# Tycro-Games/Raytracer-VoxPopuli

Measured on AMD Instinct MI355X. Metric: Mray/s (primary+shadow) at 1920×1080, 1024³ world; 1/2/4/8-GPU, higher is better.
Workload: dtype f32

## Files before the change

include/vpx.h:

```cpp
#ifndef VPX_H_
#define VPX_H_

#include <stddef.h>
#include <stdint.h>

#ifdef __cplusplus
extern "C" {
#endif

#define VPX_ABI_VERSION 2

#define VPX_OK 0
#define VPX_E_INVALID (-1)
#define VPX_E_DEVICE (-2)
#define VPX_E_NOMEM (-3)
#define VPX_E_STATE (-4)

#define VPX_MAT_NON_METAL_WHITE 0
#define VPX_MAT_NON_METAL_PINK 4
#define VPX_MAT_METAL_HIGH 5
#define VPX_MAT_METAL_LOW 7
#define VPX_MAT_GLASS 8
#define VPX_MAT_SMOKE_LOW_DENSITY 9
#define VPX_MAT_SMOKE_PLAYER 14
// ... 118 lines not shown
const char* vpx_last_error(const vpx_ctx* ctx);
int vpx_abi_version(void);
int vpx_set_stream(vpx_ctx* ctx, void* hip_stream);
int vpx_synchronize(vpx_ctx* ctx);
int vpx_set_pipeline(vpx_ctx* ctx, uint32_t depth);

int vpx_upload_grid(vpx_ctx* ctx, uint32_t grid_id, const uint8_t* cells, uint32_t n);
int vpx_generate_tiled_grid(vpx_ctx* ctx, uint32_t grid_id, uint32_t n, const uint8_t* model,
                            uint32_t mx, uint32_t my, uint32_t mz,
                            uint32_t px, uint32_t py, uint32_t pz, uint32_t ground);
int vpx_grid_fill(vpx_ctx* ctx, uint32_t grid_id, uint8_t value);
int vpx_grid_write_box(vpx_ctx* ctx, uint32_t grid_id, const uint8_t* src, uint32_t x0, uint32_t y0,
                       uint32_t z0, uint32_t dx, uint32_t dy, uint32_t dz);
int vpx_grid_emissive_sphere(vpx_ctx* ctx, uint32_t grid_id, uint8_t mat, float radius);
int vpx_grid_checksum(vpx_ctx* ctx, uint32_t grid_id, uint64_t* out);
int vpx_grid_axis_planes(vpx_ctx* ctx, uint32_t grid_id, uint16_t* out, uint64_t count);
int vpx_set_volumes(vpx_ctx* ctx, const vpx_volume* volumes, uint32_t count);
int vpx_set_materials(vpx_ctx* ctx, const vpx_material* materials, uint32_t count);
int vpx_set_lights(vpx_ctx* ctx,
                   const vpx_point_light* points, uint32_t n_points,
                   const vpx_spot_light* spots, uint32_t n_spots,
                   const vpx_area_light* areas, uint32_t n_areas,
                   const vpx_dir_light* dir);
int vpx_set_shapes(vpx_ctx* ctx, const vpx_sphere* spheres, uint32_t n_spheres,
                   const vpx_triangle* triangles, uint32_t n_triangles);
int vpx_set_camera(vpx_ctx* ctx, const vpx_camera* camera);
int vpx_set_sky(vpx_ctx* ctx, const float* rgb, uint32_t width, uint32_t height,
                float hdr_contribution);

#define VPX_ARITH_EXACT 0u
// ... 104 lines not shown
```

raytracer-voxpopuli_amd/abi.py:

```python
import ctypes as C
import os

import numpy as np

HERE = os.path.dirname(os.path.abspath(__file__))
LIB_PATH = os.path.join(HERE, "libvpx_hip.so")
ABI_VERSION = 2

VPX_OK = 0
VPX_E_INVALID, VPX_E_DEVICE, VPX_E_NOMEM, VPX_E_STATE = -1, -2, -3, -4
VPX_FLAG_AA = 0x1
VPX_FLAG_DOF = 0x2
VPX_FLAG_NO_TONEMAP = 0x4
VPX_ARITH_EXACT, VPX_ARITH_X86_HOST = 0, 1
VPX_FLAG_SKY = 0x8
MAT_NONE = 255
SKY_DEFAULT = (0.392, 0.584, 0.829)

f3 = C.c_float * 3


class Volume(C.Structure):
    _fields_ = [("grid_id", C.c_uint32), ("reserved", C.c_uint32), ("matrix", C.c_float * 16),
                ("inv_matrix", C.c_float * 16), ("b0", f3), ("b1", f3)]
# ... 102 lines not shown
    "vpx_create": (C.c_int, [C.c_int, C.POINTER(C.c_void_p)]),
    "vpx_create_multi": (C.c_int, [C.POINTER(C.c_int), C.c_int, C.POINTER(C.c_void_p)]),
    "vpx_destroy": (C.c_int, [C.c_void_p]),
    "vpx_last_error": (C.c_char_p, [C.c_void_p]),
    "vpx_abi_version": (C.c_int, []),
    "vpx_set_stream": (C.c_int, [C.c_void_p, C.c_void_p]),
    "vpx_synchronize": (C.c_int, [C.c_void_p]),
    "vpx_set_pipeline": (C.c_int, [C.c_void_p, C.c_uint32]),
    "vpx_gl_register_buffer": (C.c_int, [C.c_void_p, C.c_uint]),
    "vpx_gl_map": (C.c_int, [C.c_void_p, C.POINTER(C.c_void_p), C.POINTER(C.c_size_t)]),
    "vpx_gl_unmap": (C.c_int, [C.c_void_p]),
    "vpx_upload_grid": (C.c_int, [C.c_void_p, C.c_uint32, C.c_void_p, C.c_uint32]),
    "vpx_generate_tiled_grid": (C.c_int, [C.c_void_p, C.c_uint32, C.c_uint32, C.c_void_p] + [C.c_uint32] * 7),
    "vpx_grid_checksum": (C.c_int, [C.c_void_p, C.c_uint32, C.POINTER(C.c_uint64)]),
    "vpx_grid_axis_planes": (C.c_int, [C.c_void_p, C.c_uint32, C.c_void_p, C.c_uint64]),
    "vpx_set_volumes": (C.c_int, [C.c_void_p, C.POINTER(Volume), C.c_uint32]),
    "vpx_set_materials": (C.c_int, [C.c_void_p, C.POINTER(Material), C.c_uint32]),
    "vpx_set_lights": (C.c_int, [C.c_void_p, C.POINTER(PointLight), C.c_uint32, C.POINTER(SpotLight), C.c_uint32,
                                 C.POINTER(AreaLight), C.c_uint32, C.POINTER(DirLight)]),
    "vpx_set_shapes": (C.c_int, [C.c_void_p, C.POINTER(Sphere), C.c_uint32, C.POINTER(Triangle), C.c_uint32]),
    "vpx_set_camera": (C.c_int, [C.c_void_p, C.POINTER(Camera)]),
    "vpx_set_sky": (C.c_int, [C.c_void_p, C.c_void_p, C.c_uint32, C.c_uint32, C.c_float]),
    "vpx_render": (C.c_int, [C.c_void_p, C.POINTER(FrameParams), C.c_void_p, C.c_void_p, C.POINTER(Stats)]),
    "vpx_render_tiles": (C.c_int, [C.c_void_p, C.POINTER(FrameParams), C.c_uint32, C.c_uint32, C.c_uint32,
                                   C.c_uint32, C.c_void_p, C.POINTER(Stats)]),
    "vpx_render_tiles_accum": (C.c_int, [C.c_void_p, C.POINTER(FrameParams), C.c_uint32, C.c_uint32, C.c_uint32,
                                         C.c_uint32, C.c_void_p, C.c_void_p, C.POINTER(Stats)]),
    "vpx_composite_rgb8": (C.c_int, [C.c_void_p, C.POINTER(FrameParams), C.c_uint32, C.c_uint32, C.c_uint32,
                                     C.c_void_p, C.c_void_p]),
    "vpx_render_window": (C.c_int, [C.c_void_p, C.POINTER(FrameParams), C.c_uint32, C.c_void_p, C.c_void_p]),
# ... 87 lines not shown
```

raytracer-voxpopuli_amd/context.py:

```python
import ctypes as C

import numpy as np

from . import abi


class Context:
    def __init__(self, device=0, devices=None):
        self.lib = abi.load_library()
        h = C.c_void_p()
        if devices is not None:
            arr = (C.c_int * len(devices))(*[int(d) for d in devices])
            rc = self.lib.vpx_create_multi(arr, len(devices), C.byref(h))
            if rc != abi.VPX_OK:
                raise abi.VpxError(f"vpx_create_multi(devices={list(devices)}) failed ({rc})")
            device = int(devices[0])
        else:
            rc = self.lib.vpx_create(int(device), C.byref(h))
            if rc != abi.VPX_OK:
                raise abi.VpxError(f"vpx_create(device={device}) failed ({rc}): no usable HIP device")
        self.h = h
        self.device = device
        self.devices = list(devices) if devices is not None else [device]
        self.scene = None
# ... 78 lines not shown
        self._chk(self.lib.vpx_grid_emissive_sphere(self.h, grid_id, int(mat), float(radius)),
                  "vpx_grid_emissive_sphere")

    def grid_checksum(self, grid_id=0):
        out = C.c_uint64()
        self._chk(self.lib.vpx_grid_checksum(self.h, grid_id, C.byref(out)), "vpx_grid_checksum")
        return out.value

    def grid_axis_planes(self, grid_id, n):
        nb2 = ((n + 3) // 4 + 3) // 4
        out = np.zeros((24, 64 * nb2 ** 3), np.uint16)
        self._chk(self.lib.vpx_grid_axis_planes(self.h, grid_id, out.ctypes.data_as(C.c_void_p), out.size),
                  "vpx_grid_axis_planes")
        return out

    def render(self, params, accum_ptr, rgb_ptr=None, stats=False):
        st = abi.Stats() if stats else None
        self._chk(self.lib.vpx_render(self.h, C.byref(params), C.c_void_p(accum_ptr), C.c_void_p(rgb_ptr or 0),
                                      C.byref(st) if st is not None else None), "vpx_render")
        return st

    def render_reproject(self, params, prev, history_ptr, rgb_ptr=None, stats=False):
        st = abi.Stats() if stats else None
        self._chk(self.lib.vpx_render_reproject(self.h, C.byref(params), C.byref(prev), C.c_void_p(history_ptr),
                                                C.c_void_p(rgb_ptr or 0), C.byref(st) if st is not None else None),
                  "vpx_render_reproject")
        return st

    def render_tiles(self, params, rank, n_ranks, packed_ptr, stats=False, tile=16):
        st = abi.Stats() if stats else None
# ... 104 lines not shown
```

raytracer-voxpopuli_amd/csrc/vpx_kernels.hip:

```cpp
#include <hip/hip_runtime.h>
#include <hip/hip_gl_interop.h>
#include <rccl/rccl.h>

#include <algorithm>
#include <cmath>
#include <cstdio>
#include <cstdlib>
#include <cstring>
#include <string>
#include <array>
#include <atomic>
#include <vector>

#include "vpx_wavefront.hpp"

using namespace vpx;

namespace {

constexpr int kTile = 16;
#ifndef VPX_SPLIT_PRIMARY
#define VPX_SPLIT_PRIMARY 1
#endif
#ifndef VPX_DEFER_INSTANCES
// ... 332 lines not shown
                               uint32_t nb3, uint8_t* __restrict__ dfp) {
    const uint64_t plane = (uint64_t)nb2 * nb2 * nb2 * 64;
    for (uint64_t s = (uint64_t)blockIdx.x * blockDim.x + threadIdx.x; s < plane; s += (uint64_t)gridDim.x * blockDim.x) {
        const uint64_t parent = s >> 6;
        const uint32_t j = (uint32_t)(s & 63u);
        const uint32_t bx = (uint32_t)(parent % nb2) * 4 + (j & 3u);
        const uint32_t by = (uint32_t)((parent / nb2) % nb2) * 4 + ((j >> 2) & 3u);
        const uint32_t bz = (uint32_t)(parent / ((uint64_t)nb2 * nb2)) * 4 + (j >> 4);
        const bool occ = (l2[skip::blk_index(bx >> 2, by >> 2, bz >> 2, nb3)] >> ((bx & 3u) | ((by & 3u) << 2) | ((bz & 3u) << 4))) & 1ull;
        const uint64_t m = occ ? 0ull : l1[s];
#pragma unroll
        for (uint32_t o = 0; o < 8; ++o) dfp[o * plane + s] = (uint8_t)(m >> (8 * o));
    }
}

__global__ void build_axis_k(const uint8_t* __restrict__ dfp, uint32_t nb1, uint32_t nb2, uint16_t* __restrict__ dfa) {
    const uint64_t plane = (uint64_t)nb2 * nb2 * nb2 * 64;
    const uint64_t total = plane * 24;
    for (uint64_t t = (uint64_t)blockIdx.x * blockDim.x + threadIdx.x; t < total; t += (uint64_t)gridDim.x * blockDim.x) {
        const uint32_t oa = (uint32_t)(t / plane);
        const uint64_t s = t - (uint64_t)oa * plane;
        const uint32_t o = oa / 3u, a = oa - o * 3u;
        const uint64_t parent = s >> 6;
        const uint32_t j = (uint32_t)(s & 63u);
        const uint32_t bx = (uint32_t)(parent % nb2) * 4 + (j & 3u);
        const uint32_t by = (uint32_t)((parent / nb2) % nb2) * 4 + ((j >> 2) & 3u);
        const uint32_t bz = (uint32_t)(parent / ((uint64_t)nb2 * nb2)) * 4 + (j >> 4);
        const uint8_t* pl = dfp + (uint64_t)o * plane;
        const uint32_t k = pl[s];
        auto cube = [&](uint32_t x, uint32_t y, uint32_t z) -> uint32_t { return pl[skip::blk_index(x, y, z, nb2)]; };
        dfa[t] = k ? (uint16_t)(k | skip::axis_len(bx, by, bz, o, a, k, nb1, cube) << 8) : (uint16_t)0;
    }
}

__global__ void write_box_k(uint8_t* __restrict__ grid, uint32_t n, const uint8_t* __restrict__ src, uint32_t x0,
                            uint32_t y0, uint32_t z0, uint32_t dx, uint32_t dy, uint32_t dz) {
    const uint64_t total = (uint64_t)dx * dy * dz;
    const uint64_t n64 = n;
    for (uint64_t i = (uint64_t)blockIdx.x * blockDim.x + threadIdx.x; i < total; i += (uint64_t)gridDim.x * blockDim.x) {
        const uint64_t x = i % dx, y = (i / dx) % dy, z = i / ((uint64_t)dx * dy);
        grid[(x0 + x) + (y0 + y) * n64 + (z0 + z) * n64 * n64] = src[i];
    }
}

__global__ void emissive_sphere_k(uint8_t* __restrict__ grid, uint32_t n, uint8_t mat, float radius, uint32_t x0,
                                  uint32_t cnt) {
// ... 854 lines not shown
        VPX_HIP(c, sync_all(c));
        (void)hipFree(g.ptr);
        (void)hipFree(g.l1);
        (void)hipFree(g.l2);
        (void)hipFree(g.dfp);
        g.ptr = nullptr, g.l1 = nullptr, g.l2 = nullptr, g.dfp = nullptr;
    }
    g.n = n;
    g.nb1 = (n + 3) / 4;
    g.nb2 = (g.nb1 + 3) / 4;
    g.nb3 = (g.nb2 + 3) / 4;
    if (!g.ptr) {
        VPX_HIP(c, hipMalloc(&g.ptr, bytes));
        VPX_HIP(c, hipMalloc(&g.l1, sizeof(uint64_t) * (size_t)g.nb2 * g.nb2 * g.nb2 * 64));
        VPX_HIP(c, hipMalloc(&g.l2, sizeof(uint64_t) * (size_t)g.nb3 * g.nb3 * g.nb3 * 64));
        VPX_HIP(c, hipMalloc(&g.dfp, (8 + 2 * 24) * g.plane()));
    }
    return sync_grids(c);
}

static int build_df(vpx_ctx* c, const vpx_ctx::GridBuf& g) {
    const uint64_t threads = (uint64_t)g.nb1 * g.nb1 * 8;
    const unsigned blocks = (unsigned)((threads + 255) / 256);
    for (uint32_t s = 3 * (g.nb1 - 1) + 1; s-- > 0;) {
        hipLaunchKernelGGL(df_plane_k, dim3(blocks), dim3(256), 0, c->stream, (uint8_t*)g.l1, g.l2, g.nb1, g.nb2, g.nb3, s);
        VPX_HIP(c, hipGetLastError());
    }
    hipLaunchKernelGGL(build_planes_k, dim3(2048), dim3(256), 0, c->stream, g.l1, g.l2, g.nb2, g.nb3, g.dfp);
    VPX_HIP(c, hipGetLastError());
    hipLaunchKernelGGL(build_axis_k, dim3(8192), dim3(256), 0, c->stream, g.dfp, g.nb1, g.nb2, (uint16_t*)(g.dfp + 8 * g.plane()));
    VPX_HIP(c, hipGetLastError());
    return VPX_OK;
}

static int build_masks(vpx_ctx* c, uint32_t id) {
    auto& g = c->grids[id];
    hipLaunchKernelGGL(build_l1_k, dim3(2048), dim3(256), 0, c->stream, g.ptr, g.n, g.nb1, g.nb2, g.l1);
    VPX_HIP(c, hipGetLastError());
    hipLaunchKernelGGL(build_up_k, dim3(512), dim3(256), 0, c->stream, g.l1, g.nb2, g.nb3, g.l2);
    VPX_HIP(c, hipGetLastError());
    if (int r = build_df(c, g)) return r;
    VPX_HIP(c, sync_all(c));
    return VPX_OK;
}

// ... 105 lines not shown
int vpx_grid_checksum(vpx_ctx* c, uint32_t id, uint64_t* out) {
    VPX_GROUP_FIRST(c, vpx_grid_checksum(m_, id, out));
    if (!c || !out) return fail(c, VPX_E_INVALID, "null argument");
    if (id >= c->grids.size() || !c->grids[id].ptr) return fail(c, VPX_E_INVALID, "unknown grid");
    const uint64_t count = (uint64_t)c->grids[id].n * c->grids[id].n * c->grids[id].n;
    VPX_HIP(c, hipMemsetAsync(c->d_sum, 0, sizeof(unsigned long long), c->stream));
    hipLaunchKernelGGL(checksum_k, dim3(2048), dim3(256), 0, c->stream, c->grids[id].ptr, count, c->d_sum);
    VPX_HIP(c, hipGetLastError());
    unsigned long long h = 0;
    VPX_HIP(c, hipMemcpyAsync(&h, c->d_sum, sizeof(h), hipMemcpyDeviceToHost, c->stream));
    VPX_HIP(c, sync_all(c));
    *out = (uint64_t)h;
    return VPX_OK;
}

int vpx_grid_axis_planes(vpx_ctx* c, uint32_t id, uint16_t* out, uint64_t count) {
    VPX_GROUP_FIRST(c, vpx_grid_axis_planes(m_, id, out, count));
    if (!c || !out) return fail(c, VPX_E_INVALID, "null argument");
    if (id >= c->grids.size() || !c->grids[id].ptr) return fail(c, VPX_E_INVALID, "unknown grid");
    const auto& g = c->grids[id];
    if (count > 24 * g.plane()) return fail(c, VPX_E_INVALID, "more words than the axis planes hold");
    VPX_HIP(c, hipMemcpyAsync(out, g.dfp + 8 * g.plane(), count * sizeof(uint16_t), hipMemcpyDeviceToHost, c->stream));
    VPX_HIP(c, sync_all(c));
    return VPX_OK;
}

struct VolBox {
    float4 lo, hi;
};
static VolBox volume_bounds(const vpx_volume& v) {
    const float* m = v.inv_matrix;
    const double a[3][3] = {{m[0], m[1], m[2]}, {m[4], m[5], m[6]}, {m[8], m[9], m[10]}};
    const double det = a[0][0] * (a[1][1] * a[2][2] - a[1][2] * a[2][1]) -
                       a[0][1] * (a[1][0] * a[2][2] - a[1][2] * a[2][0]) +
                       a[0][2] * (a[1][0] * a[2][1] - a[1][1] * a[2][0]);
    const VolBox none{make_float4(-INFINITY, -INFINITY, -INFINITY, 0.f), make_float4(INFINITY, INFINITY, INFINITY, 0.f)};
    if (!(std::fabs(det) > 1e-30)) return none;
    double r[3][3];
// ... 940 lines not shown
```

raytracer-voxpopuli_amd/csrc/vpx_skip.hpp:

```cpp
#pragma once

#include <stdint.h>

#ifndef __HIP_DEVICE_COMPILE__
#include <cstring>
#endif

#if defined(__HIPCC__)
#define VPX_HD __host__ __device__ __forceinline__
#else
#define VPX_HD inline
#endif

namespace vpx {
namespace skip {

VPX_HD uint32_t fbits(float f) {
#if defined(__HIP_DEVICE_COMPILE__)
    return __float_as_uint(f);
#else
    uint32_t u;
    std::memcpy(&u, &f, 4);
    return u;
#endif
// ... 167 lines not shown

}
}

namespace vpx {
namespace skip {

struct GridView {
    const uint8_t* cells;
    const uint64_t* l1;
    const uint64_t* l2;
    uint32_t n, nb1, nb2, nb3;
    const uint8_t* dfp;
    uint64_t plane;
    const uint16_t* dfa;
};

struct Walk {
    uint32_t X, Y, Z;
    float t, tx, ty, tz;
    float dx, dy, dz;
    int32_t sx, sy, sz;
    uint32_t osh;
    uint64_t m1, m2;
};

VPX_HD void walk_begin(Walk& w) {
    w.m1 = w.m2 = 0ull;
    w.osh = ((w.sx < 0 ? 1u : 0u) | (w.sy < 0 ? 2u : 0u) | (w.sz < 0 ? 4u : 0u)) * 8u;
}
// ... 65 lines not shown
    const uint32_t bx = w.X >> 2, by = w.Y >> 2, bz = w.Z >> 2, np = g.nb2;
#if defined(__HIP_DEVICE_COMPILE__)
    const uint32_t parent = opar + __umul24(bz >> 2, __umul24(np, np)) + __umul24(by >> 2, np) + (bx >> 2);
#else
    const uint32_t parent = opar + (bz >> 2) * np * np + (by >> 2) * np + (bx >> 2);
#endif
    const uint64_t i = (uint64_t)parent << 6 | ((bx & 3u) | ((by & 3u) << 2) | ((bz & 3u) << 4));
#if defined(__HIP_DEVICE_COMPILE__)
    const uint32_t k = ((const __attribute__((address_space(1))) uint8_t*)g.dfp)[i];
#else
    const uint32_t k = g.dfp[i];
#endif
    return classify_dfp_byte<MINC>(w, g, k);
}
VPX_HD uint32_t plane_parent(const GridView& g, uint32_t o) { return o * (g.nb2 * g.nb2 * g.nb2); }
VPX_HD uint32_t dom_axis(const Walk& w) {
    return w.dx <= w.dy ? (w.dx <= w.dz ? 0u : 2u) : (w.dy <= w.dz ? 1u : 2u);
}
template <uint32_t MINC = kMinCube, uint32_t MINL = 2>
VPX_HD int classify_axis_o(Walk& w, const GridView& g, uint32_t apar) {
    const uint32_t bx = w.X >> 2, by = w.Y >> 2, bz = w.Z >> 2, np = g.nb2;
#if defined(__HIP_DEVICE_COMPILE__)
    const uint32_t parent = apar + __umul24(bz >> 2, __umul24(np, np)) + __umul24(by >> 2, np) + (bx >> 2);
#else
    const uint32_t parent = apar + (bz >> 2) * np * np + (by >> 2) * np + (bx >> 2);
#endif
    const uint64_t i = (uint64_t)parent << 6 | ((bx & 3u) | ((by & 3u) << 2) | ((bz & 3u) << 4));
#if defined(__HIP_DEVICE_COMPILE__)
    const uint32_t kl = ((const __attribute__((address_space(1))) uint16_t*)g.dfa)[i];
#else
    const uint32_t kl = g.dfa[i];
#endif
    if (kl == 0u) {
        w.m1 = load_mask(g.l1, blk_index(bx, by, bz, np));
        const uint32_t cb = (w.X & 3u) | ((w.Y & 3u) << 2) | ((w.Z & 3u) << 4);
        return ((w.m1 >> cb) & 1ull) ? 0 : 1;
    }
    w.m1 = kl;
    return (((kl & 255u) >= MINC) | ((kl >> 8) >= MINL)) ? 2 : 3;
}
VPX_HD uint32_t len_dfa(const Walk& w) { return ((uint32_t)w.m1 >> 8) & 255u; }
VPX_HD uint32_t cube_l1(const Walk& w) { return (uint32_t)(w.m1 >> w.osh) & 255u; }
VPX_HD uint32_t cube_dfp(const Walk& w) { return (uint32_t)w.m1 & 255u; }
VPX_HD void df_box(const Walk& w, uint32_t n, uint32_t k, uint32_t lo[3], uint32_t hi[3]) {
    const uint32_t k4 = k * 4u;
    const uint32_t c[3] = {w.X, w.Y, w.Z};
    const int32_t sg[3] = {w.sx, w.sy, w.sz};
    for (int k = 0; k < 3; ++k) {
        const uint32_t b = c[k] & ~3u;
        const uint32_t up = b + k4 - 1u, dn = b + 4u > k4 ? b + 4u - k4 : 0u;
        lo[k] = sg[k] > 0 ? c[k] : dn;
        hi[k] = sg[k] > 0 ? (up < n - 1u ? up : n - 1u) : c[k];
    }
}

VPX_HD void df_box_axis(const Walk& w, uint32_t n, uint32_t k, uint32_t L, uint32_t axis, uint32_t lo[3], uint32_t hi[3]) {
    const uint32_t c[3] = {w.X, w.Y, w.Z};
    const int32_t sg[3] = {w.sx, w.sy, w.sz};
    for (uint32_t q = 0; q < 3; ++q) {
        const uint32_t e4 = (q == axis ? L : k) * 4u;
        const uint32_t b = c[q] & ~3u;
        const uint32_t up = b + e4 - 1u, dn = b + 4u > e4 ? b + 4u - e4 : 0u;
        lo[q] = sg[q] > 0 ? c[q] : dn;
        hi[q] = sg[q] > 0 ? (up < n - 1u ? up : n - 1u) : c[q];
    }
}

VPX_HD bool step1_commit(Walk& w, uint32_t n, bool ax, bool ay, bool az) {
    w.X += ax ? (uint32_t)w.sx : 0u;
    w.Y += ay ? (uint32_t)w.sy : 0u;
    w.Z += az ? (uint32_t)w.sz : 0u;
    w.tx = ax ? w.tx + w.dx : w.tx;
    w.ty = ay ? w.ty + w.dy : w.ty;
    w.tz = az ? w.tz + w.dz : w.tz;
    const uint32_t m = w.X > w.Y ? w.X : w.Y;
// ... 271 lines not shown
        w.tx = axis_at(ax, w.tx, nx), w.ty = axis_at(ay, w.ty, ny), w.tz = axis_at(az, w.tz, nz);
        w.X += nx * (uint32_t)w.sx;
        w.Y += ny * (uint32_t)w.sy;
        w.Z += nz * (uint32_t)w.sz;
        cells += nx + ny + nz;
        return 0;
    }
    const uint32_t cx = a == 0 ? lx : axis_count(ax, w.tx, vs, true, lx);
    const uint32_t cy = a == 1 ? ly : axis_count(ay, w.ty, vs, a == 2, ly);
    const uint32_t cz = a == 2 ? lz : axis_count(az, w.tz, vs, false, lz);
    cells += 1u + (nx < cx ? nx : cx) + (ny < cy ? ny : cy) + (nz < cz ? nz : cz);
    return 1;
}

VPX_HD bool walk_skip(const GridView& g, Walk& w, float bound, uint32_t& cells) {
    const bool axes = g.dfa != nullptr;
    const uint32_t axis = dom_axis(w);
    const uint32_t apar = plane_parent(g, (w.osh >> 3) * 3u + axis);
    for (;;) {
        if (!(w.t < bound)) return false;
        const int cls = axes ? classify_axis_o(w, g, apar) : classify(w, g);
        if (cls == 0) {
            ++cells;
            return true;
        }
        if (cls == 2) {
            uint32_t lo[3], hi[3];
            if (axes) df_box_axis(w, g.n, cube_dfp(w), len_dfa(w), axis, lo, hi);
            else df_box(w, g.n, cube_l1(w), lo, hi);
            if (skip_box_lean(w, lo, hi, bound, cells) == 1) return false;
        }
        ++cells;
        if (!step1(w, g.n)) return false;
    }
}

template <class Occ, class Get>
VPX_HD uint8_t df_value(uint32_t x, uint32_t y, uint32_t z, uint32_t o, uint32_t nb1, Occ occ, Get get) {
    const int32_t s[3] = {(o & 1u) ? -1 : 1, (o & 2u) ? -1 : 1, (o & 4u) ? -1 : 1};
    uint32_t mn = 255;
    for (uint32_t j = 1; j < 8; ++j) {
        const uint32_t a = x + ((j & 1u) ? (uint32_t)s[0] : 0u), b = y + ((j & 2u) ? (uint32_t)s[1] : 0u),
                       c = z + ((j & 4u) ? (uint32_t)s[2] : 0u);
// ... 3 lines not shown
    return (uint8_t)(mn < 255u ? mn + 1u : 255u);
}

template <class Cube>
VPX_HD uint32_t axis_len(uint32_t x, uint32_t y, uint32_t z, uint32_t o, uint32_t a, uint32_t k, uint32_t nb1, Cube cube) {
    const uint32_t e = ((o >> a) & 1u) ? ~0u : 1u;
    uint32_t p[3] = {x, y, z};
    uint32_t L = k;
    while (L < 255u) {
        p[a] += e;
        if (p[a] >= nb1) return 255u;
        if (cube(p[0], p[1], p[2]) < k) break;
        ++L;
    }
    return L;
}

#if !defined(__HIP_DEVICE_COMPILE__)
inline void build_masks_host(const uint8_t* cells, uint32_t n, uint64_t* l1, uint64_t* l2) {
    const uint32_t nb1 = (n + 3) / 4, nb2 = (nb1 + 3) / 4, nb3 = (nb2 + 3) / 4;
    std::memset(l1, 0, 8ull * nb2 * nb2 * nb2 * 64);
    std::memset(l2, 0, 8ull * nb3 * nb3 * nb3 * 64);
    for (uint64_t z = 0; z < n; ++z)
        for (uint64_t y = 0; y < n; ++y)
            for (uint64_t x = 0; x < n; ++x)
                if (cells[x + y * n + z * (uint64_t)n * n] != 255)
                    l1[blk_index((uint32_t)x >> 2, (uint32_t)y >> 2, (uint32_t)z >> 2, nb2)] |=
                        1ull << ((x & 3) + 4 * (y & 3) + 16 * (z & 3));
    for (uint32_t z = 0; z < nb1; ++z)
        for (uint32_t y = 0; y < nb1; ++y)
// ... 35 lines not shown
    const uint64_t plane = 64ull * nb2 * nb2 * nb2;
    std::memset(dfa, 0, 2 * 24 * plane);
    for (uint32_t o = 0; o < 8; ++o) {
        const uint8_t* pl = dfp + o * plane;
        auto cube = [&](uint32_t x, uint32_t y, uint32_t z) -> uint32_t { return pl[blk_index(x, y, z, nb2)]; };
        for (uint32_t z = 0; z < nb1; ++z)
            for (uint32_t y = 0; y < nb1; ++y)
                for (uint32_t x = 0; x < nb1; ++x) {
                    const uint32_t b = blk_index(x, y, z, nb2), k = pl[b];
                    if (!k) continue;
                    for (uint32_t a = 0; a < 3; ++a)
                        dfa[(o * 3 + a) * plane + b] = (uint16_t)(k | axis_len(x, y, z, o, a, k, nb1, cube) << 8);
                }
    }
}
#endif

}
}
```

raytracer-voxpopuli_amd/csrc/vpx_trace.hpp:

```cpp
#pragma once

#include <hip/hip_runtime.h>
#include <stdint.h>

#include "../../include/vpx.h"
#include "vpx_skip.hpp"
#include "vpx_x86.hpp"

namespace vpx {

constexpr uint32_t kNone = 255u;
constexpr float kPi = 3.14159265358979323846264f;
constexpr float kBig = 1e34f;
constexpr int kMaxLevels = 16;

struct DevGrid {
    const uint8_t* cells;
    const uint64_t* l1;
    const uint64_t* l2;
    uint32_t n;
    uint32_t nb1;
    uint32_t nb2;
    uint32_t nb3;
    const uint8_t* dfp;
// ... 313 lines not shown
    const float mind = smin(smin(d.x, d.y), d.z);
    const f3 sg = dsign(r.D) * 2.0f - mk(1.f, 1.f, 1.f);
    const f3 nn = mk(mind == d.x ? sg.x : 0.0f, mind == d.y ? sg.y : 0.0f, mind == d.z ? sg.z : 0.0f);
    return normalize(xform_vec(nn, matrix));
}

__device__ __forceinline__ uint32_t uni(uint32_t v) { return __builtin_amdgcn_readfirstlane(v); }
template <class T>
__device__ __forceinline__ T* uni_ptr(T* p) {
    const uint64_t v = (uint64_t)p;
    return (T*)(((uint64_t)uni((uint32_t)(v >> 32)) << 32) | uni((uint32_t)v));
}
__device__ __forceinline__ skip::GridView grid_view(const DevGrid& g) {
    const uint8_t* dfp = uni_ptr(g.dfp);
    return skip::GridView{uni_ptr(g.cells), uni_ptr(g.l1), uni_ptr(g.l2), uni(g.n), uni(g.nb1), uni(g.nb2),
                          uni(g.nb3),       dfp,            g.plane,        (const uint16_t*)(dfp + 8u * g.plane)};
}
__device__ __forceinline__ skip::Walk to_walk(const Dda& s) {
    skip::Walk w;
    w.X = s.X, w.Y = s.Y, w.Z = s.Z;
    w.t = s.t;
    w.tx = s.tmax.x, w.ty = s.tmax.y, w.tz = s.tmax.z;
    w.dx = s.tdelta.x, w.dy = s.tdelta.y, w.dz = s.tdelta.z;
    w.sx = s.sx, w.sy = s.sy, w.sz = s.sz;
    skip::walk_begin(w);
    return w;
}

constexpr uint32_t kSkipwNearest = 1, kSkipwBounce = 2, kSkipwShadow = 4;
#ifndef VPX_MINC_NEAREST
#define VPX_MINC_NEAREST 2
#endif
constexpr uint32_t kMincNearest = VPX_MINC_NEAREST, kMincBounce = 2, kMincShadow = 1;
#ifndef VPX_AXIS_BOXES
#define VPX_AXIS_BOXES 1
#endif
#ifndef VPX_AXIS_MINLEN
#define VPX_AXIS_MINLEN 2u
#endif
#define VPX_RUN_AXIS ((VPX_AXIS_BOXES ? 1u : 0u) << 19 | VPX_AXIS_MINLEN << 20)
#ifndef VPX_RUN_NEAREST
#define VPX_RUN_NEAREST (3u | 3u << 8 | 1u << 17 | 1u << 18 | VPX_RUN_AXIS)
#endif
constexpr uint32_t kRunNearest = VPX_RUN_NEAREST;
#ifndef VPX_RUN_BOUNCE
#define VPX_RUN_BOUNCE (4u | 1u << 8 | 0u << 17 | 1u << 18 | VPX_RUN_AXIS)
#endif
constexpr uint32_t kRunBounce = VPX_RUN_BOUNCE;
#ifndef VPX_RUN_SHADOW
#define VPX_RUN_SHADOW (3u | 1u << 8 | 1u << 17 | 0u << 18 | VPX_RUN_AXIS)
#endif
constexpr uint32_t kRunShadow = VPX_RUN_SHADOW;
#ifndef VPX_RUN_FRAME_NEAREST
#define VPX_RUN_FRAME_NEAREST (3u | 4u << 8 | 1u << 17 | 1u << 18 | VPX_RUN_AXIS)
#endif
constexpr uint32_t kRunFrameNearest = VPX_RUN_FRAME_NEAREST;
#ifndef VPX_RUN_FRAME_SHADOW
#define VPX_RUN_FRAME_SHADOW (3u | 2u << 8 | 1u << 17 | 1u << 18 | VPX_RUN_AXIS)
#endif
constexpr uint32_t kRunFrameShadow = VPX_RUN_FRAME_SHADOW;
#ifndef VPX_RUN_SHADOW_POOL
#define VPX_RUN_SHADOW_POOL (3u | 1u << 8 | 1u << 17 | 1u << 18 | VPX_RUN_AXIS)
#endif
#ifndef VPX_SKIPW_SHADOW_POOL
#define VPX_SKIPW_SHADOW_POOL 4u
#endif
#ifndef VPX_MINC_SHADOW_POOL
#define VPX_MINC_SHADOW_POOL 1u
#endif
constexpr uint32_t kRunShadowPool = VPX_RUN_SHADOW_POOL, kSkipwShadowPool = VPX_SKIPW_SHADOW_POOL,
                   kMincShadowPool = VPX_MINC_SHADOW_POOL;
#ifdef VPX_ASM_MARKS
#define VPX_MARK(s) asm volatile("; MARK " s)
#else
#define VPX_MARK(s)
#endif

// ... 3 lines not shown
#else
#define VPX_PH(...)
#endif

constexpr int kWalkStep = 0, kWalkSkip = 1, kWalkMiss = 2, kWalkHit = 3;
template <int PHK, uint32_t SKIPW, uint32_t MINC, uint32_t RUN, bool POOL = false>
__device__ __forceinline__ bool walk_wave(const skip::GridView& g, skip::Walk& w, float bound, uint32_t& cells,
                                          int* pmode = nullptr, uint32_t leave = 65u) {
    enum : int { kStep = kWalkStep, kSkip = kWalkSkip, kMiss = kWalkMiss, kHit = kWalkHit };
    constexpr int kRun = (int)(RUN & 255u);
    constexpr int kPasses = (int)((RUN >> 8) & 255u);
    constexpr bool kSeg2Branch = (RUN >> 17) & 1u;
    constexpr bool kMin2 = (RUN >> 18) & 1u;
    constexpr bool kAxis = (RUN >> 19) & 1u;
    constexpr uint32_t kMinLen = (RUN >> 20) & 15u;
    static_assert(SKIPW > 0 && kRun > 0 && kPasses > 0, "walk_wave: skip weight, run cap and passes");
    static_assert(!kAxis || kMinLen > 0, "walk_wave: the axis boxes' minimum length");
    const uint32_t opar = skip::plane_parent(g, kAxis ? (w.osh >> 3) * 3u + skip::dom_axis(w) : w.osh >> 3);
    int mode = POOL ? *pmode : kStep;
    VPX_PH(uint64_t cs = 0, ck = 0, ns = 0, nk = 0, ls = 0, lk = 0, fb = 0, cf = 0;)
    for (;;) {
        VPX_PH(uint64_t t0 = __builtin_amdgcn_s_memtime();)
        for (;;) {
            const uint64_t stepping = __ballot(mode == kStep);
            if (!stepping) break;
            const uint32_t nskip = (uint32_t)__popcll(__ballot(mode == kSkip));
            if ((uint32_t)__popcll(stepping) * SKIPW < nskip) break;
            if (POOL && 64u - (uint32_t)__popcll(stepping) - nskip >= leave) goto pool_out;
            VPX_PH(++ns; ls += __popcll(stepping); cf += __popcll(__ballot(mode >= kMiss));)
            VPX_MARK("step body");
// ... 26 lines not shown
                    }
                }
            }
        }
        VPX_MARK("step phase end");
        VPX_PH(uint64_t t1 = __builtin_amdgcn_s_memtime(); cs += t1 - t0;)
        const uint64_t skipping = __ballot(mode == kSkip);
        if (!skipping) {
            if (!__ballot(mode == kStep)) break;
            continue;
        }
        VPX_PH(++nk; lk += __popcll(skipping);)
        VPX_MARK("skip phase");
        if (mode == kSkip) {
            uint32_t lo[3], hi[3];
            if (kAxis) skip::df_box_axis(w, g.n, skip::cube_dfp(w), skip::len_dfa(w), skip::dom_axis(w), lo, hi);
            else skip::df_box(w, g.n, skip::cube_dfp(w), lo, hi);
            const int sr = skip::skip_box_lean<kSeg2Branch>(w, lo, hi, bound, cells);
            VPX_MARK("skip end");
            VPX_PH(fb += __popcll(__ballot(sr == 2));)
            if (sr == 1) {
                mode = kMiss;
            } else {
                ++cells;
                mode = skip::step1<kMin2>(w, g.n) ? kStep : kMiss;
            }
        }
        VPX_PH(ck += __builtin_amdgcn_s_memtime() - t1;)
    }
    if (POOL) {
    pool_out:
        *pmode = mode;
// ... 762 lines not shown
```

Measured before the change: 5914.

## Widen axis distance-field boxes along a second axis using 32-bit plane words

Axis-plane entries grow from 16 to 32 bits. A new build pass computes, for each block, how far the empty box can extend along the two non-dominant axes, and stores that in the upper bytes. During traversal, the skip box is stretched along the ray's secondary axis by that width, so each skip covers more empty space. The cost is double the memory for the axis planes, wider loads in the classify step, an extra build kernel, and an asm barrier that recomputes the axis locally to limit register pressure.

```diff
diff --git a/include/vpx.h b/include/vpx.h
--- a/include/vpx.h
+++ b/include/vpx.h
@@ -156,6 +156,7 @@
                        uint32_t z0, uint32_t dx, uint32_t dy, uint32_t dz);
 int vpx_grid_emissive_sphere(vpx_ctx* ctx, uint32_t grid_id, uint8_t mat, float radius);
 int vpx_grid_checksum(vpx_ctx* ctx, uint32_t grid_id, uint64_t* out);
+int vpx_grid_wide_planes(vpx_ctx* ctx, uint32_t grid_id, uint32_t* out, uint64_t count);
 int vpx_grid_axis_planes(vpx_ctx* ctx, uint32_t grid_id, uint16_t* out, uint64_t count);
 int vpx_set_volumes(vpx_ctx* ctx, const vpx_volume* volumes, uint32_t count);
 int vpx_set_materials(vpx_ctx* ctx, const vpx_material* materials, uint32_t count);
diff --git a/raytracer-voxpopuli_amd/abi.py b/raytracer-voxpopuli_amd/abi.py
--- a/raytracer-voxpopuli_amd/abi.py
+++ b/raytracer-voxpopuli_amd/abi.py
@@ -140,6 +140,7 @@
     "vpx_generate_tiled_grid": (C.c_int, [C.c_void_p, C.c_uint32, C.c_uint32, C.c_void_p] + [C.c_uint32] * 7),
     "vpx_grid_checksum": (C.c_int, [C.c_void_p, C.c_uint32, C.POINTER(C.c_uint64)]),
     "vpx_grid_axis_planes": (C.c_int, [C.c_void_p, C.c_uint32, C.c_void_p, C.c_uint64]),
+    "vpx_grid_wide_planes": (C.c_int, [C.c_void_p, C.c_uint32, C.c_void_p, C.c_uint64]),
     "vpx_set_volumes": (C.c_int, [C.c_void_p, C.POINTER(Volume), C.c_uint32]),
     "vpx_set_materials": (C.c_int, [C.c_void_p, C.POINTER(Material), C.c_uint32]),
     "vpx_set_lights": (C.c_int, [C.c_void_p, C.POINTER(PointLight), C.c_uint32, C.POINTER(SpotLight), C.c_uint32,
diff --git a/raytracer-voxpopuli_amd/context.py b/raytracer-voxpopuli_amd/context.py
--- a/raytracer-voxpopuli_amd/context.py
+++ b/raytracer-voxpopuli_amd/context.py
@@ -116,6 +116,13 @@
                   "vpx_grid_axis_planes")
         return out
 
+    def grid_wide_planes(self, grid_id, n):
+        nb2 = ((n + 3) // 4 + 3) // 4
+        out = np.zeros((24, 64 * nb2 ** 3), np.uint32)
+        self._chk(self.lib.vpx_grid_wide_planes(self.h, grid_id, out.ctypes.data_as(C.c_void_p), out.size),
+                  "vpx_grid_wide_planes")
+        return out
+
     def render(self, params, accum_ptr, rgb_ptr=None, stats=False):
         st = abi.Stats() if stats else None
         self._chk(self.lib.vpx_render(self.h, C.byref(params), C.c_void_p(accum_ptr), C.c_void_p(rgb_ptr or 0),
diff --git a/raytracer-voxpopuli_amd/csrc/vpx_kernels.hip b/raytracer-voxpopuli_amd/csrc/vpx_kernels.hip
--- a/raytracer-voxpopuli_amd/csrc/vpx_kernels.hip
+++ b/raytracer-voxpopuli_amd/csrc/vpx_kernels.hip
@@ -370,7 +370,7 @@
     }
 }
 
-__global__ void build_axis_k(const uint8_t* __restrict__ dfp, uint32_t nb1, uint32_t nb2, uint16_t* __restrict__ dfa) {
+__global__ void build_axis_k(const uint8_t* __restrict__ dfp, uint32_t nb1, uint32_t nb2, uint32_t* __restrict__ dfw) {
     const uint64_t plane = (uint64_t)nb2 * nb2 * nb2 * 64;
     const uint64_t total = plane * 24;
     for (uint64_t t = (uint64_t)blockIdx.x * blockDim.x + threadIdx.x; t < total; t += (uint64_t)gridDim.x * blockDim.x) {
@@ -385,7 +385,27 @@
         const uint8_t* pl = dfp + (uint64_t)o * plane;
         const uint32_t k = pl[s];
         auto cube = [&](uint32_t x, uint32_t y, uint32_t z) -> uint32_t { return pl[skip::blk_index(x, y, z, nb2)]; };
-        dfa[t] = k ? (uint16_t)(k | skip::axis_len(bx, by, bz, o, a, k, nb1, cube) << 8) : (uint16_t)0;
+        dfw[t] = k ? k | skip::axis_len(bx, by, bz, o, a, k, nb1, cube) << 8 : 0u;
+    }
+}
+
+__global__ void build_wide_k(uint16_t* dfh, uint32_t nb1, uint32_t nb2) {
+    const uint64_t plane = (uint64_t)nb2 * nb2 * nb2 * 64;
+    const uint64_t total = plane * 24;
+    for (uint64_t t = (uint64_t)blockIdx.x * blockDim.x + threadIdx.x; t < total; t += (uint64_t)gridDim.x * blockDim.x) {
+        const uint32_t oa = (uint32_t)(t / plane);
+        const uint64_t s = t - (uint64_t)oa * plane;
+        const uint32_t o = oa / 3u, a = oa - o * 3u;
+        const uint64_t parent = s >> 6;
+        const uint32_t j = (uint32_t)(s & 63u);
+        const uint32_t bx = (uint32_t)(parent % nb2) * 4 + (j & 3u);
+        const uint32_t by = (uint32_t)((parent / nb2) % nb2) * 4 + ((j >> 2) & 3u);
+        const uint32_t bz = (uint32_t)(parent / ((uint64_t)nb2 * nb2)) * 4 + (j >> 4);
+        const uint16_t* pl = dfh + 2 * (uint64_t)oa * plane;
+        const uint32_t kl = pl[2 * s];
+        if (!kl || bx >= nb1 || by >= nb1 || bz >= nb1) continue;
+        auto word = [&](uint32_t x, uint32_t y, uint32_t z) -> uint32_t { return pl[2 * (uint64_t)skip::blk_index(x, y, z, nb2)]; };
+        dfh[2 * t + 1] = (uint16_t)skip::axis_wids(bx, by, bz, o, a, kl & 255u, kl >> 8, nb1, word);
     }
 }
 
@@ -1270,7 +1290,7 @@
         VPX_HIP(c, hipMalloc(&g.ptr, bytes));
         VPX_HIP(c, hipMalloc(&g.l1, sizeof(uint64_t) * (size_t)g.nb2 * g.nb2 * g.nb2 * 64));
         VPX_HIP(c, hipMalloc(&g.l2, sizeof(uint64_t) * (size_t)g.nb3 * g.nb3 * g.nb3 * 64));
-        VPX_HIP(c, hipMalloc(&g.dfp, (8 + 2 * 24) * g.plane()));
+        VPX_HIP(c, hipMalloc(&g.dfp, (8 + 4 * 24) * g.plane()));
     }
     return sync_grids(c);
 }
@@ -1284,7 +1304,9 @@
     }
     hipLaunchKernelGGL(build_planes_k, dim3(2048), dim3(256), 0, c->stream, g.l1, g.l2, g.nb2, g.nb3, g.dfp);
     VPX_HIP(c, hipGetLastError());
-    hipLaunchKernelGGL(build_axis_k, dim3(8192), dim3(256), 0, c->stream, g.dfp, g.nb1, g.nb2, (uint16_t*)(g.dfp + 8 * g.plane()));
+    hipLaunchKernelGGL(build_axis_k, dim3(8192), dim3(256), 0, c->stream, g.dfp, g.nb1, g.nb2, (uint32_t*)(g.dfp + 8 * g.plane()));
+    VPX_HIP(c, hipGetLastError());
+    hipLaunchKernelGGL(build_wide_k, dim3(8192), dim3(256), 0, c->stream, (uint16_t*)(g.dfp + 8 * g.plane()), g.nb1, g.nb2);
     VPX_HIP(c, hipGetLastError());
     return VPX_OK;
 }
@@ -1420,14 +1442,25 @@
     return VPX_OK;
 }
 
+int vpx_grid_wide_planes(vpx_ctx* c, uint32_t id, uint32_t* out, uint64_t count) {
+    VPX_GROUP_FIRST(c, vpx_grid_wide_planes(m_, id, out, count));
+    if (!c || !out) return fail(c, VPX_E_INVALID, "null argument");
+    if (id >= c->grids.size() || !c->grids[id].ptr) return fail(c, VPX_E_INVALID, "unknown grid");
+    const auto& g = c->grids[id];
+    if (count > 24 * g.plane()) return fail(c, VPX_E_INVALID, "more words than the axis planes hold");
+    VPX_HIP(c, hipMemcpyAsync(out, g.dfp + 8 * g.plane(), count * sizeof(uint32_t), hipMemcpyDeviceToHost, c->stream));
+    VPX_HIP(c, sync_all(c));
+    return VPX_OK;
+}
+
 int vpx_grid_axis_planes(vpx_ctx* c, uint32_t id, uint16_t* out, uint64_t count) {
     VPX_GROUP_FIRST(c, vpx_grid_axis_planes(m_, id, out, count));
     if (!c || !out) return fail(c, VPX_E_INVALID, "null argument");
     if (id >= c->grids.size() || !c->grids[id].ptr) return fail(c, VPX_E_INVALID, "unknown grid");
-    const auto& g = c->grids[id];
-    if (count > 24 * g.plane()) return fail(c, VPX_E_INVALID, "more words than the axis planes hold");
-    VPX_HIP(c, hipMemcpyAsync(out, g.dfp + 8 * g.plane(), count * sizeof(uint16_t), hipMemcpyDeviceToHost, c->stream));
-    VPX_HIP(c, sync_all(c));
+    if (count > 24 * c->grids[id].plane()) return fail(c, VPX_E_INVALID, "more words than the axis planes hold");
+    std::vector<uint32_t> words(count);
+    if (int r = vpx_grid_wide_planes(c, id, words.data(), count)) return r;
+    for (uint64_t i = 0; i < count; ++i) out[i] = (uint16_t)words[i];
     return VPX_OK;
 }
 
diff --git a/raytracer-voxpopuli_amd/csrc/vpx_skip.hpp b/raytracer-voxpopuli_amd/csrc/vpx_skip.hpp
--- a/raytracer-voxpopuli_amd/csrc/vpx_skip.hpp
+++ b/raytracer-voxpopuli_amd/csrc/vpx_skip.hpp
@@ -205,6 +205,7 @@
     const uint8_t* dfp;
     uint64_t plane;
     const uint16_t* dfa;
+    const uint32_t* dfw;
 };
 
 struct Walk {
@@ -300,9 +301,12 @@
     return classify_dfp_byte<MINC>(w, g, k);
 }
 VPX_HD uint32_t plane_parent(const GridView& g, uint32_t o) { return o * (g.nb2 * g.nb2 * g.nb2); }
-VPX_HD uint32_t dom_axis(const Walk& w) {
-    return w.dx <= w.dy ? (w.dx <= w.dz ? 0u : 2u) : (w.dy <= w.dz ? 1u : 2u);
-}
+VPX_HD uint32_t dom_axis(float dx, float dy, float dz) { return dx <= dy ? (dx <= dz ? 0u : 2u) : (dy <= dz ? 1u : 2u); }
+VPX_HD uint32_t dom_axis(const Walk& w) { return dom_axis(w.dx, w.dy, w.dz); }
+VPX_HD uint32_t sec_axis(uint32_t a, float dx, float dy, float dz) {
+    return a == 0u ? (dy <= dz ? 1u : 2u) : (a == 1u ? (dx <= dz ? 0u : 2u) : (dx <= dy ? 0u : 1u));
+}
+VPX_HD uint32_t sec_axis(const Walk& w) { return sec_axis(dom_axis(w), w.dx, w.dy, w.dz); }
 template <uint32_t MINC = kMinCube, uint32_t MINL = 2>
 VPX_HD int classify_axis_o(Walk& w, const GridView& g, uint32_t apar) {
     const uint32_t bx = w.X >> 2, by = w.Y >> 2, bz = w.Z >> 2, np = g.nb2;
@@ -313,9 +317,9 @@
 #endif
     const uint64_t i = (uint64_t)parent << 6 | ((bx & 3u) | ((by & 3u) << 2) | ((bz & 3u) << 4));
 #if defined(__HIP_DEVICE_COMPILE__)
-    const uint32_t kl = ((const __attribute__((address_space(1))) uint16_t*)g.dfa)[i];
-#else
-    const uint32_t kl = g.dfa[i];
+    const uint32_t kl = ((const __attribute__((address_space(1))) uint32_t*)g.dfw)[i];
+#else
+    const uint32_t kl = g.dfw ? g.dfw[i] : g.dfa[i];
 #endif
     if (kl == 0u) {
         w.m1 = load_mask(g.l1, blk_index(bx, by, bz, np));
@@ -323,9 +327,12 @@
         return ((w.m1 >> cb) & 1ull) ? 0 : 1;
     }
     w.m1 = kl;
-    return (((kl & 255u) >= MINC) | ((kl >> 8) >= MINL)) ? 2 : 3;
+    return (((kl & 255u) >= MINC) | (((kl >> 8) & 255u) >= MINL)) ? 2 : 3;
 }
 VPX_HD uint32_t len_dfa(const Walk& w) { return ((uint32_t)w.m1 >> 8) & 255u; }
+VPX_HD uint32_t wid_dfw(const Walk& w, uint32_t axis, uint32_t sec) {
+    return ((uint32_t)w.m1 >> (sec < 3u - axis - sec ? 16u : 24u)) & 255u;
+}
 VPX_HD uint32_t cube_l1(const Walk& w) { return (uint32_t)(w.m1 >> w.osh) & 255u; }
 VPX_HD uint32_t cube_dfp(const Walk& w) { return (uint32_t)w.m1 & 255u; }
 VPX_HD void df_box(const Walk& w, uint32_t n, uint32_t k, uint32_t lo[3], uint32_t hi[3]) {
@@ -340,11 +347,12 @@
     }
 }
 
-VPX_HD void df_box_axis(const Walk& w, uint32_t n, uint32_t k, uint32_t L, uint32_t axis, uint32_t lo[3], uint32_t hi[3]) {
+VPX_HD void df_box_axis(const Walk& w, uint32_t n, uint32_t k, uint32_t L, uint32_t axis, uint32_t lo[3], uint32_t hi[3],
+                        uint32_t sec = 3u, uint32_t M = 0u) {
     const uint32_t c[3] = {w.X, w.Y, w.Z};
     const int32_t sg[3] = {w.sx, w.sy, w.sz};
     for (uint32_t q = 0; q < 3; ++q) {
-        const uint32_t e4 = (q == axis ? L : k) * 4u;
+        const uint32_t e4 = (q == axis ? L : (q == sec ? M : k)) * 4u;
         const uint32_t b = c[q] & ~3u;
         const uint32_t up = b + e4 - 1u, dn = b + 4u > e4 ? b + 4u - e4 : 0u;
         lo[q] = sg[q] > 0 ? c[q] : dn;
@@ -646,8 +654,8 @@
 }
 
 VPX_HD bool walk_skip(const GridView& g, Walk& w, float bound, uint32_t& cells) {
-    const bool axes = g.dfa != nullptr;
-    const uint32_t axis = dom_axis(w);
+    const bool wide = g.dfw != nullptr, axes = wide || g.dfa != nullptr;
+    const uint32_t axis = dom_axis(w), sec = wide ? sec_axis(w) : 3u;
     const uint32_t apar = plane_parent(g, (w.osh >> 3) * 3u + axis);
     for (;;) {
         if (!(w.t < bound)) return false;
@@ -658,7 +666,7 @@
         }
         if (cls == 2) {
             uint32_t lo[3], hi[3];
-            if (axes) df_box_axis(w, g.n, cube_dfp(w), len_dfa(w), axis, lo, hi);
+            if (axes) df_box_axis(w, g.n, cube_dfp(w), len_dfa(w), axis, lo, hi, sec, wide ? wid_dfw(w, axis, sec) : 0u);
             else df_box(w, g.n, cube_l1(w), lo, hi);
             if (skip_box_lean(w, lo, hi, bound, cells) == 1) return false;
         }
@@ -692,6 +700,49 @@
         ++L;
     }
     return L;
+}
+
+#ifndef VPX_WID_CAP
+#define VPX_WID_CAP 255u
+#endif
+template <class Word>
+VPX_HD uint32_t axis_wid(const uint32_t p[3], uint32_t o, uint32_t a, uint32_t b, uint32_t c, uint32_t k, uint32_t L, uint32_t nb1,
+                         Word word) {
+    const uint32_t ea = ((o >> a) & 1u) ? ~0u : 1u, eb = ((o >> b) & 1u) ? ~0u : 1u, ec = ((o >> c) & 1u) ? ~0u : 1u;
+    const uint32_t top = k > VPX_WID_CAP ? k : VPX_WID_CAP;
+    uint32_t q[3];
+    uint32_t M = k;
+    while (M < top) {
+        q[b] = p[b] + eb * M;
+        if (q[b] >= nb1) return top;
+        uint32_t layers = 1u;
+        for (uint32_t m = 0; m < k;) {
+            q[c] = p[c] + ec * m;
+            if (q[c] >= nb1) break;
+            uint32_t rows = 1u;
+            for (uint32_t i = 0; i < L;) {
+                q[a] = p[a] + ea * i;
+                if (q[a] >= nb1) break;
+                const uint32_t w = word(q[0], q[1], q[2]);
+                if (!w) return M;
+                const uint32_t k2 = w & 255u, L2 = (w >> 8) & 255u;
+                if (i == 0u && L2 >= L) {
+                    rows = k2;
+                    if (m == 0u && k2 >= k) layers = k2;
+                }
+                i += L2;
+            }
+            m += rows;
+        }
+        M += layers;
+    }
+    return top;
+}
+template <class Word>
+VPX_HD uint32_t axis_wids(uint32_t x, uint32_t y, uint32_t z, uint32_t o, uint32_t a, uint32_t k, uint32_t L, uint32_t nb1, Word word) {
+    const uint32_t p[3] = {x, y, z};
+    const uint32_t b = a == 0u ? 1u : 0u, c = a == 2u ? 1u : 2u;
+    return axis_wid(p, o, a, b, c, k, L, nb1, word) | axis_wid(p, o, a, c, b, k, L, nb1, word) << 8;
 }
 
 #if !defined(__HIP_DEVICE_COMPILE__)
@@ -757,7 +808,33 @@
                 }
     }
 }
-#endif
-
-}
-}
+
+inline void build_wide_planes_host(const uint8_t* dfp, uint32_t n, uint32_t* dfw) {
+    const uint32_t nb1 = (n + 3) / 4, nb2 = (nb1 + 3) / 4;
+    const uint64_t plane = 64ull * nb2 * nb2 * nb2;
+    std::memset(dfw, 0, 4 * 24 * plane);
+    for (uint32_t oa = 0; oa < 24; ++oa) {
+        const uint8_t* pl = dfp + (oa / 3u) * plane;
+        auto cube = [&](uint32_t x, uint32_t y, uint32_t z) -> uint32_t { return pl[blk_index(x, y, z, nb2)]; };
+        for (uint32_t z = 0; z < nb1; ++z)
+            for (uint32_t y = 0; y < nb1; ++y)
+                for (uint32_t x = 0; x < nb1; ++x) {
+                    const uint32_t b = blk_index(x, y, z, nb2), k = pl[b];
+                    if (k) dfw[oa * plane + b] = k | axis_len(x, y, z, oa / 3u, oa % 3u, k, nb1, cube) << 8;
+                }
+    }
+    for (uint32_t oa = 0; oa < 24; ++oa) {
+        uint32_t* pl = dfw + oa * plane;
+        auto word = [&](uint32_t x, uint32_t y, uint32_t z) -> uint32_t { return pl[blk_index(x, y, z, nb2)] & 0xffffu; };
+        for (uint32_t z = 0; z < nb1; ++z)
+            for (uint32_t y = 0; y < nb1; ++y)
+                for (uint32_t x = 0; x < nb1; ++x) {
+                    const uint32_t b = blk_index(x, y, z, nb2), kl = pl[b] & 0xffffu;
+                    if (kl) pl[b] = kl | axis_wids(x, y, z, oa / 3u, oa % 3u, kl & 255u, kl >> 8, nb1, word) << 16;
+                }
+    }
+}
+#endif
+
+}
+}
diff --git a/raytracer-voxpopuli_amd/csrc/vpx_trace.hpp b/raytracer-voxpopuli_amd/csrc/vpx_trace.hpp
--- a/raytracer-voxpopuli_amd/csrc/vpx_trace.hpp
+++ b/raytracer-voxpopuli_amd/csrc/vpx_trace.hpp
@@ -351,7 +351,7 @@
 __device__ __forceinline__ skip::GridView grid_view(const DevGrid& g) {
     const uint8_t* dfp = uni_ptr(g.dfp);
     return skip::GridView{uni_ptr(g.cells), uni_ptr(g.l1), uni_ptr(g.l2), uni(g.n), uni(g.nb1), uni(g.nb2),
-                          uni(g.nb3),       dfp,            g.plane,        (const uint16_t*)(dfp + 8u * g.plane)};
+                          uni(g.nb3),       dfp,            g.plane,        nullptr,  (const uint32_t*)(dfp + 8u * g.plane)};
 }
 __device__ __forceinline__ skip::Walk to_walk(const Dda& s) {
     skip::Walk w;
@@ -375,29 +375,37 @@
 #ifndef VPX_AXIS_MINLEN
 #define VPX_AXIS_MINLEN 2u
 #endif
-#define VPX_RUN_AXIS ((VPX_AXIS_BOXES ? 1u : 0u) << 19 | VPX_AXIS_MINLEN << 20)
+#ifndef VPX_WIDE_BOXES
+#define VPX_WIDE_BOXES 1
+#endif
+#ifdef VPX_LOCAL_AXES
+#define VPX_RUN_LOCAL(on) ((VPX_LOCAL_AXES ? 1u : 0u) << 25)
+#else
+#define VPX_RUN_LOCAL(on) ((on) << 25)
+#endif
+#define VPX_RUN_AXIS ((VPX_AXIS_BOXES ? 1u : 0u) << 19 | VPX_AXIS_MINLEN << 20 | (VPX_AXIS_BOXES && VPX_WIDE_BOXES ? 1u : 0u) << 24)
 #ifndef VPX_RUN_NEAREST
-#define VPX_RUN_NEAREST (3u | 3u << 8 | 1u << 17 | 1u << 18 | VPX_RUN_AXIS)
+#define VPX_RUN_NEAREST (3u | 3u << 8 | 1u << 17 | 1u << 18 | VPX_RUN_AXIS | VPX_RUN_LOCAL(1u))
 #endif
 constexpr uint32_t kRunNearest = VPX_RUN_NEAREST;
 #ifndef VPX_RUN_BOUNCE
-#define VPX_RUN_BOUNCE (4u | 1u << 8 | 0u << 17 | 1u << 18 | VPX_RUN_AXIS)
+#define VPX_RUN_BOUNCE (4u | 1u << 8 | 0u << 17 | 1u << 18 | VPX_RUN_AXIS | VPX_RUN_LOCAL(0u))
 #endif
 constexpr uint32_t kRunBounce = VPX_RUN_BOUNCE;
 #ifndef VPX_RUN_SHADOW
-#define VPX_RUN_SHADOW (3u | 1u << 8 | 1u << 17 | 0u << 18 | VPX_RUN_AXIS)
+#define VPX_RUN_SHADOW (3u | 1u << 8 | 1u << 17 | 0u << 18 | VPX_RUN_AXIS | VPX_RUN_LOCAL(1u))
 #endif
 constexpr uint32_t kRunShadow = VPX_RUN_SHADOW;
 #ifndef VPX_RUN_FRAME_NEAREST
-#define VPX_RUN_FRAME_NEAREST (3u | 4u << 8 | 1u << 17 | 1u << 18 | VPX_RUN_AXIS)
+#define VPX_RUN_FRAME_NEAREST (3u | 4u << 8 | 1u << 17 | 1u << 18 | VPX_RUN_AXIS | VPX_RUN_LOCAL(1u))
 #endif
 constexpr uint32_t kRunFrameNearest = VPX_RUN_FRAME_NEAREST;
 #ifndef VPX_RUN_FRAME_SHADOW
-#define VPX_RUN_FRAME_SHADOW (3u | 2u << 8 | 1u << 17 | 1u << 18 | VPX_RUN_AXIS)
+#define VPX_RUN_FRAME_SHADOW (3u | 2u << 8 | 1u << 17 | 1u << 18 | VPX_RUN_AXIS | VPX_RUN_LOCAL(1u))
 #endif
 constexpr uint32_t kRunFrameShadow = VPX_RUN_FRAME_SHADOW;
 #ifndef VPX_RUN_SHADOW_POOL
-#define VPX_RUN_SHADOW_POOL (3u | 1u << 8 | 1u << 17 | 1u << 18 | VPX_RUN_AXIS)
+#define VPX_RUN_SHADOW_POOL (3u | 1u << 8 | 1u << 17 | 1u << 18 | VPX_RUN_AXIS | VPX_RUN_LOCAL(1u))
 #endif
 #ifndef VPX_SKIPW_SHADOW_POOL
 #define VPX_SKIPW_SHADOW_POOL 4u
@@ -431,6 +439,9 @@
     constexpr bool kMin2 = (RUN >> 18) & 1u;
     constexpr bool kAxis = (RUN >> 19) & 1u;
     constexpr uint32_t kMinLen = (RUN >> 20) & 15u;
+    constexpr bool kWide = (RUN >> 24) & 1u;
+    constexpr bool kLocal = (RUN >> 25) & 1u;
+    static_assert(!kWide || kAxis, "walk_wave: wide boxes are axis boxes");
     static_assert(SKIPW > 0 && kRun > 0 && kPasses > 0, "walk_wave: skip weight, run cap and passes");
     static_assert(!kAxis || kMinLen > 0, "walk_wave: the axis boxes' minimum length");
     const uint32_t opar = skip::plane_parent(g, kAxis ? (w.osh >> 3) * 3u + skip::dom_axis(w) : w.osh >> 3);
@@ -487,8 +498,14 @@
         VPX_MARK("skip phase");
         if (mode == kSkip) {
             uint32_t lo[3], hi[3];
-            if (kAxis) skip::df_box_axis(w, g.n, skip::cube_dfp(w), skip::len_dfa(w), skip::dom_axis(w), lo, hi);
-            else skip::df_box(w, g.n, skip::cube_dfp(w), lo, hi);
+            if (kAxis) {
+                float dx = w.dx, dy = w.dy, dz = w.dz;
+                if (kLocal) asm volatile("" : "+v"(dx), "+v"(dy), "+v"(dz));
+                const uint32_t axis = skip::dom_axis(dx, dy, dz), sec = kWide ? skip::sec_axis(axis, dx, dy, dz) : 3u;
+                skip::df_box_axis(w, g.n, skip::cube_dfp(w), skip::len_dfa(w), axis, lo, hi, sec, kWide ? skip::wid_dfw(w, axis, sec) : 0u);
+            } else {
+                skip::df_box(w, g.n, skip::cube_dfp(w), lo, hi);
+            }
             const int sr = skip::skip_box_lean<kSeg2Branch>(w, lo, hi, bound, cells);
             VPX_MARK("skip end");
             VPX_PH(fb += __popcll(__ballot(sr == 2));)
```

After: 6257 (median of 6 runs). 1.06x the previous value.
